# Da1yuqin/TCDiff

Hardware: AMD Instinct MI355X
Metric: sampled clips/sec (3 dancers x 150 frames, 1000 DDPM steps) (higher is better)
Workload: dtype bf16; 1 GPU; batch=16 clips/GPU, 3 dancers x 150 frames, 1000 DDPM steps (p_sample_loop, CFG w=2, cosine schedule), bf16, 1xMI355X; clips_per_gpu=16, ddpm_steps=1000

## Files before the change

### tcdiff_amd/csrc/chain.hip

```cpp
#include "common.h"
#include "tcdiff_hip.h"

#include "chain_core.h"

#ifdef CH_ABLATE_ROWLAT
#define CH_RP_NEXT(rp, nt) do { } while (0)
#else
#define CH_RP_NEXT(rp, nt) rp_issue(rp, nt)
#endif

template <int HH, int MT, int NT, bool SELF = false>
DEVINL void cross_attention(const f32x4_t (&qacc)[NT][MT], const tcdiff_chain_args& a, int m0, int Mv, int lblk, char* abuf,
                            int wave, int lane) {
#ifdef CH_XATT_ONEPASS
    constexpr bool PARK = !SELF;
#else
    constexpr bool PARK = false;
#endif
    constexpr bool ONEPASS = SELF || PARK;
    constexpr int NPS = ONEPASS ? 1 : (MT == 4 ? 2 : 1), NML = ONEPASS ? MT : (MT == 1 ? 1 : 2);
    lane = fresh_v(lane);
    wave = fresh_s(wave) * (NT / 4) + HH;
    const int c = lane & 15, g = lane >> 4;
    const int M = Mv, L = a.L, nkt = SELF ? a.sa_nkt : a.nkt, Lk = SELF ? a.L : a.Lk;
    const float qs = a.scale_q * CH_LOG2E;
    u32x4 qf[MT][2];
    if constexpr (SELF) {
        const u32x4* qsrc = reinterpret_cast<const u32x4*>(a.sa_q) + ((long)(lblk * 8 + wave) * 8) * 64 + lane;
#pragma unroll
        for (int mt = 0; mt < MT; ++mt)
#pragma unroll
            for (int s = 0; s < 2; ++s) qf[mt][s] = qsrc[(mt * 2 + s) * 64];
    } else {
#pragma unroll
        for (int mt = 0; mt < MT; ++mt)
#pragma unroll
            for (int s = 0; s < 2; ++s) {
                const f32x4_t lo = qacc[4 * HH + 2 * s][mt], hi = qacc[4 * HH + 2 * s + 1][mt];
                qf[mt][s][0] = pack_bf2(lo[0] * qs, lo[1] * qs);
                qf[mt][s][1] = pack_bf2(lo[2] * qs, lo[3] * qs);
                qf[mt][s][2] = pack_bf2(hi[0] * qs, hi[1] * qs);
                qf[mt][s][3] = pack_bf2(hi[2] * qs, hi[3] * qs);
            }
    }
    char* qpark = abuf + (CH_H1C - CH_ABUF) + wave * 8192 + lane * 16;
    if constexpr (PARK) {
#pragma unroll
        for (int mt = 0; mt < MT; ++mt)
#pragma unroll
            for (int s = 0; s < 2; ++s) *reinterpret_cast<u32x4*>(qpark + (mt * 2 + s) * 1024) = qf[mt][s];
    }
    u32x4 ones = {0x3F803F80u, 0x3F803F80u, 0x3F803F80u, 0x3F803F80u};
    asm volatile("" : "+v"(ones));
    const unsigned voff = (unsigned)lane * 16u;
    const __amdgpu_buffer_rsrc_t kr = __builtin_amdgcn_make_buffer_rsrc(const_cast<void*>(SELF ? a.sa_kf : a.kf), 0, -1, 0x00020000);
    const __amdgpu_buffer_rsrc_t vr = __builtin_amdgcn_make_buffer_rsrc(const_cast<void*>(SELF ? a.sa_vf : a.vf), 0, -1, 0x00020000);
    auto ld_tile = [&](const __amdgpu_buffer_rsrc_t& r, unsigned so, u32x4 (&f)[4]) {
#pragma unroll
        for (int i = 0; i < 4; ++i) f[i] = __builtin_bit_cast(u32x4, __builtin_amdgcn_raw_buffer_load_b128(r, voff + 1024u * i, so, 0));
    };
#pragma unroll
    for (int ps = 0; ps < NPS; ++ps) {
        int ra = m0 + 16 * NML * ps, rb = ra + 16 * NML - 1;
        ra = ra < M ? ra : M - 1;
        rb = rb < M ? rb : M - 1;
        const int sa = ra / L, sb = rb / L;
        int my_seq[NML];
#pragma unroll
        for (int ml = 0; ml < NML; ++ml) {
            int mrow = m0 + 16 * NML * ps + 16 * ml + c;
            mrow = mrow < M ? mrow : M - 1;
            my_seq[ml] = mrow / L;
        }
#pragma unroll 1
        for (int seq = sa; seq <= sb; ++seq) {
            const int kv = SELF ? seq : seq < a.n_shared ? 0 : seq - a.n_shared + (a.n_shared > 0 ? 1 : 0);
            const unsigned so0 = (unsigned)((kv * a.H + wave) * nkt) * 4096u;
            f32x4_t o[4][NML];
#pragma unroll
            for (int dt = 0; dt < 4; ++dt)
#pragma unroll
                for (int ml = 0; ml < NML; ++ml) o[dt][ml] = f32x4_t{0, 0, 0, 0};
            f32x4_t lacc[NML];
            float m_run[NML], nb[NML];
#pragma unroll
            for (int ml = 0; ml < NML; ++ml) {
                m_run[ml] = -INFINITY;
                nb[ml] = 0.0f;
                lacc[ml] = f32x4_t{0, 0, 0, 0};
            }
            u32x4 kn[4];
            ld_tile(kr, so0, kn);
#pragma unroll 1
            for (int kt = 0; kt < nkt; ++kt) {
                u32x4 kc[4], vc[4];
#pragma unroll
                for (int i = 0; i < 4; ++i) kc[i] = kn[i];
                ld_tile(vr, so0 + (unsigned)kt * 4096u, vc);
                const int nx = kt + 1 < nkt ? kt + 1 : kt;
                if constexpr (!PARK) ld_tile(kr, so0 + (unsigned)nx * 4096u, kn);
                f32x4_t s0[NML], s1[NML];
#pragma unroll
                for (int ml = 0; ml < NML; ++ml) {
                    const int mt = NML * ps + ml;
                    s0[ml] = s1[ml] = f32x4_t{nb[ml], nb[ml], nb[ml], nb[ml]};
                    u32x4 q0 = qf[mt][0], q1 = qf[mt][1];
                    if constexpr (PARK) {
                        char* qp = qpark;
                        asm volatile("" : "+v"(qp));
                        q0 = *reinterpret_cast<const u32x4*>(qp + (mt * 2) * 1024);
                        q1 = *reinterpret_cast<const u32x4*>(qp + (mt * 2 + 1) * 1024);
                    }
                    mma16(s0[ml], kc[0], q0);
                    mma16(s1[ml], kc[2], q0);
                    mma16(s0[ml], kc[1], q1);
                    mma16(s1[ml], kc[3], q1);
                }
                if constexpr (PARK) {
#pragma unroll
                    for (int ml = 0; ml < NML; ++ml) asm volatile("" : "+v"(s0[ml]), "+v"(s1[ml]));
                    ld_tile(kr, so0 + (unsigned)nx * 4096u, kn);
                }
                if (kt * 32 + 32 > Lk) {
#pragma unroll
                    for (int ml = 0; ml < NML; ++ml)
#pragma unroll
                        for (int j = 0; j < 4; ++j) {
                            if (kt * 32 + 4 * g + j >= Lk) s0[ml][j] = -INFINITY;
                            if (kt * 32 + 16 + 4 * g + j >= Lk) s1[ml][j] = -INFINITY;
                        }
                }
                float lm[NML];
                bool hot = kt == 0;
#pragma unroll
                for (int ml = 0; ml < NML; ++ml) {
                    lm[ml] = lane_max8(s0[ml], s1[ml], -INFINITY);
                    hot = hot || lm[ml] > CH_ATT_THR;
                }
                if (__builtin_amdgcn_ballot_w64(hot) != 0) {
#pragma unroll
                    for (int ml = 0; ml < NML; ++ml) {
                        const float mx = ar4_max(lm[ml]);
                        const float m_new = (kt == 0 || mx > CH_ATT_THR) ? fmaxf(m_run[ml], mx - nb[ml]) : m_run[ml];
                        const float shift = m_new + nb[ml];
                        const float alpha = __builtin_amdgcn_exp2f(m_run[ml] - m_new);
                        m_run[ml] = m_new;
                        nb[ml] = -m_new;
#pragma unroll
                        for (int j = 0; j < 4; ++j) {
                            lacc[ml][j] *= alpha;
                            s0[ml][j] -= shift;
                            s1[ml][j] -= shift;
                        }
#pragma unroll
                        for (int dt = 0; dt < 4; ++dt)
#pragma unroll
                            for (int j = 0; j < 4; ++j) o[dt][ml][j] *= alpha;
                    }
                }
#pragma unroll
                for (int ml = 0; ml < NML; ++ml) {
#pragma unroll
                    for (int j = 0; j < 4; ++j) {
                        s0[ml][j] = __builtin_amdgcn_exp2f(s0[ml][j]);
                        s1[ml][j] = __builtin_amdgcn_exp2f(s1[ml][j]);
                    }
                    u32x4 pf;
                    pf[0] = pack_bf2(s0[ml][0], s0[ml][1]);
                    pf[1] = pack_bf2(s0[ml][2], s0[ml][3]);
                    pf[2] = pack_bf2(s1[ml][0], s1[ml][1]);
                    pf[3] = pack_bf2(s1[ml][2], s1[ml][3]);
#pragma unroll
                    for (int dt = 0; dt < 4; ++dt) mma16(o[dt][ml], vc[dt], pf);
                    mma16(lacc[ml], ones, pf);
                }
            }
#pragma unroll
            for (int ml = 0; ml < NML; ++ml) {
                const float lsum = lacc[ml][0];
                if (my_seq[ml] == seq) {
                    const float inv = __builtin_amdgcn_rcpf(lsum);
                    const int mt = NML * ps + ml;
#pragma unroll
                    for (int dt = 0; dt < 4; ++dt) {
                        uint2 pk;
                        pk.x = pack_bf2(o[dt][ml][0] * inv, o[dt][ml][1] * inv);
                        pk.y = pack_bf2(o[dt][ml][2] * inv, o[dt][ml][3] * inv);
                        *reinterpret_cast<uint2*>(abuf + wave * 8192 + act_wr_off(lane, dt) + mt * 2048) = pk;
                    }
                }
            }
        }
    }
}

#ifdef CH_STAMP
#ifndef CH_STAMP_BLOCK
#define CH_STAMP_BLOCK 0
#endif
#define CH_T(i) do { if (m0 == 64 * CH_STAMP_BLOCK && (threadIdx.x & 63) == 0 && (MODE == TC_CHAIN_B || MODE == TC_CHAIN_FULL)) \
        reinterpret_cast<unsigned long long*>(a.h_out)[(threadIdx.x >> 6) * 64 + (i)] = __builtin_amdgcn_s_memrealtime(); } while (0)
#define CH_TC(i) do { if (m0 == 64 * CH_STAMP_BLOCK && (threadIdx.x & 63) == 0 && (MODE == TC_CHAIN_B || MODE == TC_CHAIN_FULL)) \
        reinterpret_cast<unsigned long long*>(a.h_out)[(threadIdx.x >> 6) * 64 + (i)] = __builtin_amdgcn_s_memtime(); } while (0)
#else
#define CH_TC(i) do { } while (0)
#define CH_T(i) do { } while (0)
#endif

template <int MODE, int MT, int NT, int BRK>
DEVINL void chain_body(const tcdiff_chain_args& a) {
    constexpr int BR = BRK;
    constexpr int NW = ChW<NT>::NW, NTH = 64 * NW, RD = ChW<NT>::D;
    constexpr bool HAS_A = MODE == TC_CHAIN_A || MODE == TC_CHAIN_FULL || MODE == TC_CHAIN_FULL_LAST;
    constexpr bool FULL = MODE == TC_CHAIN_FULL || MODE == TC_CHAIN_FULL_LAST;
    constexpr bool LAST = MODE == TC_CHAIN_B_LAST || MODE == TC_CHAIN_FULL_LAST;
    constexpr bool FRONT = MODE == TC_CHAIN_FRONT;
    extern __shared__ __attribute__((aligned(16))) char smem[];
    const int tid = threadIdx.x, lane = tid & 63;
    const int wave = __builtin_amdgcn_readfirstlane(tid >> 6);
    const int c = lane & 15, g = lane >> 4;
    const int dn = FRONT ? a.dn : 1;
    const int dancer = FRONT ? (int)(blockIdx.x % (unsigned)dn) : 0;
    const int lblk = FRONT ? (int)(blockIdx.x / (unsigned)dn) : xcd_remap(blockIdx.x, gridDim.x);
    const bool seqcut = !FRONT && a.seq_blocks;
    const int nbs = seqcut ? (a.L + BR - 1) / BR : 1;
    const int bseq = seqcut ? lblk / nbs : 0, bis = seqcut ? lblk - bseq * nbs : 0;
    const int m0 = seqcut ? bseq * a.L + bis * BR : lblk * BR;
    CH_T(0);
    CH_TC(60);
    const int Mtot = a.M, L = a.L;
    const int M = seqcut ? (bseq + 1) * L : Mtot;
    char* abuf = smem + CH_ABUF;
    char* h1c = smem + CH_H1C;
    float* scr = reinterpret_cast<float*>(smem + CH_SCR);
    char* cfilm = smem + CH_FILM;
    char* cvec = smem + CH_VEC;

    const int seq0 = (m0 < M ? m0 : M - 1) / L;
    const int seq_last = (Mtot - 1) / L;
    const int seqb = (seq0 + 1) * L;
    struct Rows { int mc[MT], sidx[MT]; };
    auto rows = [&]() {
        Rows r;
        const int cc = fresh_v(c);
#pragma unroll
        for (int mt = 0; mt < MT; ++mt) {
            const int m = m0 + 16 * mt + cc;
            r.mc[mt] = m < M ? m : M - 1;
            r.sidx[mt] = r.mc[mt] >= seqb ? 1 : 0;
        }
        return r;
    };
    auto positions = [&](const Rows& r, int (&pos)[MT]) {
#pragma unroll
        for (int mt = 0; mt < MT; ++mt)
            pos[mt] = FRONT ? (r.mc[mt] * dn + dancer) % L : r.mc[mt] - (r.sidx[mt] ? seqb : seqb - L);
    };
    constexpr int CF = 512 / NTH, CV = (768 + NTH - 1) / NTH;
    struct Consts { f32x4_t f[CF], v[CV]; };
    auto fetch_consts = [&](const float* film, const float* const (&vec)[6]) {
        Consts k;
#pragma unroll
        for (int j = 0; j < CF; ++j) {
            const int idx = j * NTH + tid;
            int sq = seq0 + (idx >> 8);
            sq = sq < seq_last ? sq : seq_last;
            k.f[j] = film ? ld4(film + (long)sq * a.film_ld + (idx & 255) * 4) : f32x4_t{0, 0, 0, 0};
        }
#pragma unroll
        for (int j = 0; j < CV; ++j) {
            const int idx = j * NTH + tid;
            const int vi = idx >> 7;
            const float* p0 = vi == 0 ? vec[0] : vi == 1 ? vec[1] : vi == 2 ? vec[2] : vi == 3 ? vec[3] : vi == 4 ? vec[4] : vi == 5 ? vec[5] : nullptr;
            k.v[j] = p0 ? ld4(p0 + (idx & 127) * 4) : f32x4_t{0, 0, 0, 0};
        }
        return k;
    };
    auto store_consts = [&](const Consts& k) {
#pragma unroll
        for (int j = 0; j < CF; ++j) *reinterpret_cast<f32x4_t*>(cfilm + (j * NTH + tid) * 16) = k.f[j];
#pragma unroll
        for (int j = 0; j < CV; ++j)
            if (j * NTH + tid < 768) *reinterpret_cast<f32x4_t*>(cvec + (j * NTH + tid) * 16) = k.v[j];
    };
    auto vecp = [&](int slot) { return cvec + slot * 2048; };
    const float* fcb_film = FULL ? a.filmb : a.film;
    const float* n3_g = FULL ? a.n3_g : a.n2_g;
    const float* n3_b = FULL ? a.n3_b : a.n2_b;

    constexpr int NWL = 2 * MT < NW ? 2 * MT : NW;
    const bool self_att = FULL && NT == 4 && a.sa_q != nullptr;
    WStreamT<NT> ws;
    ws.rsrc = __builtin_amdgcn_make_buffer_rsrc(
        const_cast<char*>(reinterpret_cast<const char*>(a.wstream)) + ((long)dancer * NW + wave) * a.n_stages * ChW<NT>::STAGE, 0,
        a.n_stages * ChW<NT>::STAGE, 0x00020000);
    ws.voff = (unsigned)lane * 16u;
    ws.pos = 0;
    ws.last = (unsigned)a.n_stages - 1;
    auto ring_fill = [&]() {
#pragma unroll
        for (int i = 0; i < RD; ++i) ws_load(ws, i, (unsigned)i);
    };
    f32x4_t acc[NT][MT];
    if constexpr (FULL && NT == 4) {
        if (self_att) {
            cross_attention<0, MT, NT, true>(acc, a, m0, M, lblk, abuf, wave, lane);
            ring_fill();
        }
    }
    if (!self_att) {
        if (wave < NWL) {
#pragma unroll
            for (int kt = 0; kt < (FRONT ? 16 : 8); ++kt)
                stage_glds<16 * MT, NWL>(abuf + kt * 8192, reinterpret_cast<const char*>(a.A) + kt * TC_ROWB, FRONT ? 2048 : 1024, m0,
                                    M, a.a_mod, wave, lane);
        }
        ring_fill();
    }
    if (FRONT) {
        const float* const v[6] = {a.b3 + 512 * dancer, a.nn_g, a.nn_b, nullptr, nullptr, nullptr};
        store_consts(fetch_consts(nullptr, v));
    } else {
        const float* const v[6] = {nullptr, nullptr, a.n2_g, a.n2_b, nullptr, nullptr};
        store_consts(fetch_consts(a.film, v));
    }
    __builtin_amdgcn_s_waitcnt(0x0F70);
    __syncthreads();
    CH_T(1);


    float nmr[MT], rstd[MT];
    RowPipe<MT> rp;
    const long xrows = (long)Mtot * dn;
    const __amdgpu_buffer_rsrc_t xo = f32_buffer(a.xout, xrows * 512);
    Consts nxt;

    auto fc_epilogue = [&](float eps, int stamp) {
        CH_T(stamp);
        row_stats(acc, scr, wave, lane, eps, nmr, rstd);
        CH_T(stamp + 1);
        const int gg = fresh_v(g), wv = fresh_s(wave);
        const Rows rw = rows();
        const int cb0 = col_base_bytes<NT>(wv, gg);
        auto body = [&](int nt, int mt, const f32x4_t& G, const f32x4_t& Bv) {
            const f32x4_t x4 = rp.q[nt & 1][mt];
            f32x4_t o;
#pragma unroll
            for (int t = 0; t < 4; ++t) {
                float v = fmaf(fmaf(acc[nt][mt][t], rstd[mt], nmr[mt]), G[t], Bv[t]);
                v = x4[t] + v;
                acc[nt][mt][t] = v;
                o[t] = v;
            }
#ifdef CH_STORE_EARLY
            cb_store<NT>(xo, Mtot, wv, nt, rw.mc[mt], gg, o);
#endif
        };
        int fb[MT];
#pragma unroll
        for (int mt = 0; mt < MT; ++mt) {
            fb[mt] = rw.sidx[mt] * 4096 + cb0;
            asm volatile("" : "+v"(fb[mt]));
        }
#pragma unroll
        for (int nt = 0; nt < NT; ++nt) {
#pragma unroll
            for (int mt = 0; mt < MT; ++mt)
                body(nt, mt, lds4b(cfilm + fb[mt], 64 * nt), lds4b(cfilm + fb[mt], 2048 + 64 * nt));
            if (nt + 2 < NT) CH_RP_NEXT(rp, nt + 2);
            CH_FENCE();
        }
#ifndef CH_STORE_EARLY
#pragma unroll
        for (int nt = 0; nt < NT; ++nt)
#pragma unroll
            for (int mt = 0; mt < MT; ++mt) cb_store<NT>(xo, Mtot, wv, nt, rw.mc[mt], gg, acc[nt][mt]);
#endif
    };
    auto xres_start = [&]() {
        const Rows rw = rows();
        int rr[MT];
#pragma unroll
        for (int mt = 0; mt < MT; ++mt) rr[mt] = a.xres_mod > 0 ? rw.mc[mt] % a.xres_mod : rw.mc[mt];
        rp_start<NT>(rp, a.xres, rr, a.xres_rowmajor ? 0 : (a.xres_mod > 0 ? a.xres_mod : Mtot), a.xres_mod > 0 ? a.xres_mod : Mtot, wave,
                     fresh_v(g));
    };
    auto xout_start = [&]() {
        const Rows rw = rows();
        rp_start<NT>(rp, a.xout, rw.mc, Mtot, Mtot, wave, fresh_v(g));
    };
    auto rope_start = [&]() {
        const Rows rw = rows();
        int pos[MT];
        positions(rw, pos);
        rp_start<NT>(rp, a.rope, pos, a.rope_rows, a.rope_rows, wave, fresh_v(g));
    };

    if (HAS_A) {
        zero(acc);
        phase_n512<16, false, MT, NT>(acc, abuf, ws, lane);
        CH_T(2);
        xres_start();
        fc_epilogue(a.ln_eps, 40);
        CH_T(3);
        if (FULL) {
            const float* const v[6] = {nullptr, nullptr, n3_g, n3_b, nullptr, nullptr};
            nxt = fetch_consts(fcb_film, v);
        }
        rope_start();
        row_stats(acc, scr + 1024, wave, lane, a.n2_eps, nmr, rstd);
        CH_T(4);
        norm_to_lds<true, MT, NT>(acc, nmr, rstd, vecp(2), vecp(3), rp, abuf, wave, lane, nullptr);
        lds_barrier();
        CH_T(34);
        if (FULL) store_consts(nxt);
        zero(acc);
        if (!FULL) {
            phase_n512<16, false, MT, NT>(acc, abuf, ws, lane);
            store_heads<true, MT, NT>(acc, a.q_out, a.scale_q, L, a.Lp, a.H, m0, M, wave, lane, smem);
            return;
        }
#ifdef CH_STAMP
        {
            unsigned long long* sp = nullptr;
            if (m0 == 64 * CH_STAMP_BLOCK) {
                sp = reinterpret_cast<unsigned long long*>(a.h_out) + 512 + wave * 32;
                if (lane == 0) sp[16] = __builtin_amdgcn_s_memtime();
            }
            phase_n512<16, false, MT, NT>(acc, abuf, ws, lane, sp);
        }
#else
        phase_n512<16, false, MT, NT>(acc, abuf, ws, lane);
#endif
        CH_T(35);
        lds_barrier();
#ifndef CH_ABLATE_XATTN
        cross_attention<0>(acc, a, m0, M, lblk, abuf, wave, lane);
        if constexpr (NT == 8) cross_attention<1>(acc, a, m0, M, lblk, abuf, wave, lane);
#endif
        CH_T(36);
        lds_barrier();
    }
    if constexpr (!FRONT) {
    zero(acc);
    phase_n512<16, false, MT, NT>(acc, abuf, ws, lane);
    if (FULL)
        xout_start();
    else
        xres_start();
    CH_T(37);
    fc_epilogue(a.ln_eps, 42);
    CH_T(38);
    row_stats(acc, scr + 1024, wave, lane, a.n2_eps, nmr, rstd);
    CH_T(39);
    {
        const float* const v[6] = {a.b1, a.b1 + 512, nullptr, a.n4_g, a.n4_b, nullptr};
        nxt = fetch_consts(a.film3, v);
    }
    norm_to_lds<false, MT, NT>(acc, nmr, rstd, vecp(2), vecp(3), rp, abuf, wave, lane, nullptr);
    lds_barrier();
    store_consts(nxt);
    lds_barrier();
    CH_T(5);
    zero(acc);
#pragma unroll 1
    for (int ch = 0; ch < 4; ++ch) {
        f32x4_t a1[NT / 2][MT];
#pragma unroll
        for (int nt = 0; nt < NT / 2; ++nt)
#pragma unroll
            for (int mt = 0; mt < MT; ++mt) a1[nt][mt] = f32x4_t{0, 0, 0, 0};
        phase_ff1<MT, NT>(a1, abuf, ws, lane);
        CH_T(6 + 4 * ch);
        char* hb = h1c + (ch & 1) * 32768;
        CH_T(7 + 4 * ch);
        {
            const int nb = 256 * ch + 8 * NT * wave + 4 * g;
#pragma unroll
            for (int nt = 0; nt < NT / 2; ++nt) {
                const f32x4_t b4 = lds4(cvec, nb + 16 * nt);
                const int wo = ((8 * NT * wave + 16 * nt) >> 6) * 8192 + act_wr_off(lane, 0, ((8 * NT * wave + 16 * nt) & 63) >> 3);
#pragma unroll
                for (int mt = 0; mt < MT; ++mt) {
                    float v[4];
#pragma unroll
                    for (int t = 0; t < 4; ++t) v[t] = a1[nt][mt][t] + b4[t];
#ifndef CH_ABLATE_GELU
                    act4_ct<ACT_GELU>(v, ACT_GELU);
#endif
                    uint2 pk;
                    pk.x = pack_bf2(v[0], v[1]);
                    pk.y = pack_bf2(v[2], v[3]);
                    *reinterpret_cast<uint2*>(hb + wo + mt * 2048) = pk;
                }
            }
        }
        lds_barrier();
        CH_T(8 + 4 * ch);
        phase_n512<8, false, MT, NT>(acc, hb, ws, lane);
        CH_T(9 + 4 * ch);
    }
    xout_start();
    {
        const int cb2 = col_base_bytes<NT>(fresh_s(wave), fresh_v(g));
        const Rows rw = rows();
        auto body2 = [&](int nt, int mt, const f32x4_t& G, const f32x4_t& Bv) {
            const f32x4_t x4 = rp.q[nt & 1][mt];
#pragma unroll
            for (int t = 0; t < 4; ++t) acc[nt][mt][t] = x4[t] + fmaf(acc[nt][mt][t], G[t], Bv[t]);
            asm volatile("" ::"v"(acc[nt][mt][0]), "v"(acc[nt][mt][1]), "v"(acc[nt][mt][2]), "v"(acc[nt][mt][3]));
        };
        int fb2[MT];
#pragma unroll
        for (int mt = 0; mt < MT; ++mt) {
            fb2[mt] = rw.sidx[mt] * 4096 + cb2;
            asm volatile("" : "+v"(fb2[mt]));
        }
#pragma unroll
        for (int nt = 0; nt < NT; ++nt) {
#pragma unroll
            for (int mt = 0; mt < MT; ++mt)
                body2(nt, mt, lds4b(cfilm + fb2[mt], 64 * nt), lds4b(cfilm + fb2[mt], 2048 + 64 * nt));
            if (nt + 2 < NT) CH_RP_NEXT(rp, nt + 2);
            CH_FENCE();
        }
    }
    CH_T(22);
    {
        const float* const v[6] = {a.b3, a.nn_g, a.nn_b, nullptr, nullptr, nullptr};
        nxt = fetch_consts(nullptr, v);
    }
    row_stats(acc, scr, wave, lane, a.n4_eps, nmr, rstd);
    CH_T(23);
    norm_to_lds<false, MT, NT>(acc, nmr, rstd, vecp(3), vecp(4), rp, abuf, wave, lane, nullptr);
    lds_barrier();
    store_consts(nxt);
    }
    CH_T(24);
    zero(acc);
    if (FRONT)
        phase_n512<32, false, MT, NT>(acc, abuf, ws, lane);
    else if (LAST)
        phase_n512<16, true, MT, NT>(acc, abuf, ws, lane);
    else
        phase_n512<16, false, MT, NT>(acc, abuf, ws, lane);
    CH_T(25);
    lds_barrier();
#ifndef CH_STORE_EARLY
    if (!LAST) rope_start();
#endif
    {
        const int g3 = fresh_v(g);
        const int cb3 = col_base_bytes<NT>(fresh_s(wave), g3);
        const Rows rw = rows();
#pragma unroll
        for (int nt = 0; nt < NT; ++nt) {
            const int n = 16 * NT * wave + 16 * nt + 4 * g3;
            const f32x4_t b4 = lds4b(vecp(0) + cb3, 64 * nt);
#pragma unroll
            for (int mt = 0; mt < MT; ++mt) {
                f32x4_t o;
#pragma unroll
                for (int t = 0; t < 4; ++t) {
                    acc[nt][mt][t] += b4[t];
                    o[t] = acc[nt][mt][t];
                }
                if (LAST && a.out_ld > 0) {
                    if (n < a.out_ld)
                        *reinterpret_cast<f32x4_t*>(reinterpret_cast<float*>(a.h_out) + (long)rw.mc[mt] * a.out_ld + n) = o;
                } else if (LAST) {
                    uint2 pk;
                    pk.x = pack_bf2(o[0], o[1]);
                    pk.y = pack_bf2(o[2], o[3]);
                    *reinterpret_cast<uint2*>(reinterpret_cast<uint16_t*>(a.h_out) + (long)rw.mc[mt] * 512 + n) = pk;
                } else {
                    cb_store<NT>(xo, xrows, wave, nt, rw.mc[mt] * dn + dancer, g3, o);
                }
            }
            CH_FENCE();
        }
    }
    if (LAST) return;
    CH_T(26);
#ifdef CH_STORE_EARLY
    rope_start();
#endif
    row_stats(acc, scr, wave, lane, a.nn_eps, nmr, rstd);
    CH_T(27);
    norm_to_lds<true, MT, NT>(acc, nmr, rstd, vecp(1), vecp(2), rp, abuf, wave, lane, smem + CH_ABUF2);
    lds_barrier();
    CH_T(28);
    zero(acc);
    phase_n512<16, false, MT, NT>(acc, abuf, ws, lane);
    CH_T(29);
    constexpr bool FRAG = !FRONT && NT == 4;
    bool frag_out = false;
    if constexpr (FRAG) frag_out = a.qf_out != nullptr;
    if constexpr (FRAG) {
        if (frag_out) store_qfrag<MT>(acc, a.qf_out, a.scale_q, lblk, wave, lane);
    }
    if (!frag_out) store_heads<true, MT, NT>(acc, a.q_out, a.scale_q, L, a.Lp, a.H, m0, M, wave, lane, smem, dn, dancer);
    zero(acc);
    phase_n512<16, false, MT, NT>(acc, abuf, ws, lane);
    CH_T(30);
    if constexpr (FRAG) {
        if (frag_out) store_kfrag<MT>(acc, a.kf_out, bseq, bis * BR, a.out_nkt, wave, lane);
    }
    if (!frag_out) store_heads<false, MT, NT>(acc, a.k_out, 1.0f, L, a.Lp, a.H, m0, M, wave, lane, smem, dn, dancer);
    CH_T(31);
    zero(acc);
    if constexpr (FRAG) {
        if (frag_out) {
            phase_n512<16, true, MT, NT, true>(acc, smem + CH_ABUF2, ws, lane);
            CH_T(32);
            store_vfrag<MT>(acc, a.vf_out, bseq, bis * BR, a.out_nkt, L, wave, lane);
            CH_T(33);
            CH_TC(61);
            return;
        }
    }
    phase_n512<16, true, MT, NT>(acc, smem + CH_ABUF2, ws, lane);
    CH_T(32);
    store_heads<false, MT, NT>(acc, a.v_out, 1.0f, L, a.Lp, a.H, m0, M, wave, lane, smem, dn, dancer);
    CH_T(33);
    CH_TC(61);
}

template <int MODE, int MT, int NT>
__global__ __launch_bounds__(2048 / NT) void chain_kernel(tcdiff_chain_args a) {
    constexpr bool DUAL = (MODE == TC_CHAIN_FULL || MODE == TC_CHAIN_FULL_LAST) && NT == 4 && MT > 1;
    if constexpr (DUAL) {
        if (a.seq_blocks) {
            const int lblk = xcd_remap(blockIdx.x, gridDim.x);
            const int nbs = (a.L + 16 * MT - 1) / (16 * MT);
            if (a.L - (lblk % nbs) * 16 * MT <= 16) {
                chain_body<MODE, 1, NT, 16 * MT>(a);
                return;
            }
        }
    }
    chain_body<MODE, MT, NT, 16 * MT>(a);
}

static bool al16(const void* p) { return (reinterpret_cast<uintptr_t>(p) & 15) == 0; }

extern "C" int tcdiff_chain(const tcdiff_chain_args* a, hipStream_t stream) {
    if (!a || a->M <= 0 || a->L <= 0 || !a->A || !a->wstream) return TC_ERR_ARG;
    const bool front = a->mode == TC_CHAIN_FRONT;
    if (!front && a->L < 64) return TC_ERR_UNSUPPORTED;
    const int want = a->mode == TC_CHAIN_A ? 32 : a->mode == TC_CHAIN_B ? 144 : a->mode == TC_CHAIN_B_LAST ? 96 :
                     a->mode == TC_CHAIN_FULL ? 176 : a->mode == TC_CHAIN_FULL_LAST ? 128 : front ? 80 : -1;
    if (want < 0 || a->n_stages != want) return TC_ERR_ARG;
    if (a->out_ld < 0 || a->out_ld % 4 || a->out_ld > 512) return TC_ERR_ARG;
    const void* ptrs[] = {a->A, a->wstream, a->film, a->xres, a->xout, a->n2_g, a->n2_b, a->rope,
                          a->q_out, a->b1, a->film3, a->n4_g, a->n4_b, a->b3, a->nn_g, a->nn_b, a->k_out,
                          a->v_out, a->h_out, a->filmb, a->n3_g, a->n3_b, a->kf, a->vf};
    for (const void* p : ptrs)
        if (p && !al16(p)) return TC_ERR_ALIGN;
    if (front) {
        if (a->dn <= 0 || a->L % a->dn || a->L / a->dn < 8 || !a->b3 || !a->nn_g || !a->nn_b || !a->rope || !a->xout ||
            !a->q_out || !a->k_out || !a->v_out || a->H != 8 || a->Lp <= 0 || a->a_mod != 0)
            return TC_ERR_ARG;
        if ((long)a->M * 2048 >= (1L << 32)) return TC_ERR_ARG;
    } else {
        if (!a->film || a->film_ld % 4 || !a->xres || !a->xout || !a->n2_g || !a->n2_b) return TC_ERR_ARG;
        if ((long)(a->a_mod > 0 ? a->a_mod : a->M) * 1024 >= (1L << 32)) return TC_ERR_ARG;
    }
    const bool has_a = a->mode == TC_CHAIN_A || a->mode == TC_CHAIN_FULL || a->mode == TC_CHAIN_FULL_LAST;
    const bool has_b = a->mode != TC_CHAIN_A && !front;
    const bool full = a->mode == TC_CHAIN_FULL || a->mode == TC_CHAIN_FULL_LAST;
    const bool last = a->mode == TC_CHAIN_B_LAST || a->mode == TC_CHAIN_FULL_LAST;
    if (has_a && (!a->rope || a->H != 8)) return TC_ERR_ARG;
    if (a->mode == TC_CHAIN_A && (!a->q_out || a->Lp <= 0)) return TC_ERR_ARG;
    if (has_b && (!a->b1 || !a->film3 || !a->n4_g || !a->n4_b || !a->b3)) return TC_ERR_ARG;
    const bool frag_out = a->qf_out || a->kf_out || a->vf_out;
    if (has_b && !last &&
        (!a->rope || !a->nn_g || !a->nn_b || (!frag_out && (!a->q_out || !a->k_out || !a->v_out)) || a->H != 8 || a->Lp <= 0))
        return TC_ERR_ARG;
    if (last && !a->h_out) return TC_ERR_ARG;
    if (full && (!a->filmb || !a->n3_g || !a->n3_b || !a->kf || !a->vf || a->nkt <= 0 ||
                 a->Lk <= 0 || a->Lk > 32 * a->nkt || a->n_shared < 0))
        return TC_ERR_ARG;
    if (a->seq_blocks && (front || a->M % a->L)) return TC_ERR_ARG;
    if (a->sa_q && (!full || !a->seq_blocks || !a->sa_kf || !a->sa_vf || a->sa_nkt <= 0 || a->L > 32 * a->sa_nkt)) return TC_ERR_ARG;
    if (frag_out && (!a->qf_out || !a->kf_out || !a->vf_out || !has_b || last || !a->seq_blocks || a->out_nkt <= 0 ||
                     a->L > 32 * a->out_nkt))
        return TC_ERR_ARG;
    if ((a->sa_q || frag_out) && a->nw == 4) return TC_ERR_UNSUPPORTED;
    for (const void* p : {a->sa_q, a->sa_kf, a->sa_vf, (const void*)a->qf_out, (const void*)a->kf_out, (const void*)a->vf_out})
        if (p && !al16(p)) return TC_ERR_ALIGN;
    if (a->sa_q && (long)(a->M / a->L) * 8 * a->sa_nkt * 4096 >= (1L << 32)) return TC_ERR_ARG;
    static tc_dev_state dev_state;
    const int n_cu = tc_device_once(dev_state, [](int) {
#define CH_FN(M_, NT_) reinterpret_cast<const void*>(chain_kernel<M_, 4, NT_>), reinterpret_cast<const void*>(chain_kernel<M_, 2, NT_>), \
                        reinterpret_cast<const void*>(chain_kernel<M_, 1, NT_>)
        const void* fns[27] = {CH_FN(TC_CHAIN_A, 4), CH_FN(TC_CHAIN_B, 4), CH_FN(TC_CHAIN_B_LAST, 4), CH_FN(TC_CHAIN_FULL, 4),
                               CH_FN(TC_CHAIN_FULL_LAST, 4), CH_FN(TC_CHAIN_FRONT, 4),
                               CH_FN(TC_CHAIN_FULL, 8), CH_FN(TC_CHAIN_FULL_LAST, 8), CH_FN(TC_CHAIN_FRONT, 8)};
#undef CH_FN
        for (const void* f : fns) {
            hipError_t e = hipFuncSetAttribute(f, hipFuncAttributeMaxDynamicSharedMemorySize, CH_SMEM);
            if (e != hipSuccess) return e;
        }
        return hipSuccess;
    });
    if (n_cu < 0) return n_cu;
    const int units = front ? a->dn : 1;
    int mt = a->mt;
    if (mt == 0) mt = ((a->M + 15) / 16) * units <= n_cu ? 1 : ((a->M + 31) / 32) * units <= n_cu ? 2 : 4;
    if (mt != 1 && mt != 2 && mt != 4) return TC_ERR_ARG;
    dim3 grid(((a->M + 16 * mt - 1) / (16 * mt)) * units);
    if (a->seq_blocks) grid.x = (a->M / a->L) * ((a->L + 16 * mt - 1) / (16 * mt));
    if (a->nw != 0 && a->nw != 4 && a->nw != 8) return TC_ERR_ARG;
    const bool four = a->nw == 4;
    if (four && !(full || front)) return TC_ERR_UNSUPPORTED;
#define CH_LAUNCH_NT(MODE_, NT_)                                                                                              \
    do {                                                                                                                      \
        if (mt == 4) hipLaunchKernelGGL((chain_kernel<MODE_, 4, NT_>), grid, dim3(2048 / NT_), CH_SMEM, stream, *a);          \
        else if (mt == 2) hipLaunchKernelGGL((chain_kernel<MODE_, 2, NT_>), grid, dim3(2048 / NT_), CH_SMEM, stream, *a);     \
        else hipLaunchKernelGGL((chain_kernel<MODE_, 1, NT_>), grid, dim3(2048 / NT_), CH_SMEM, stream, *a);                  \
    } while (0)
#define CH_LAUNCH(MODE_) CH_LAUNCH_NT(MODE_, 4)
#define CH_LAUNCH2(MODE_) do { if (four) CH_LAUNCH_NT(MODE_, 8); else CH_LAUNCH_NT(MODE_, 4); } while (0)
    switch (a->mode) {
        case TC_CHAIN_FRONT: CH_LAUNCH2(TC_CHAIN_FRONT); break;
        case TC_CHAIN_A: CH_LAUNCH(TC_CHAIN_A); break;
        case TC_CHAIN_B: CH_LAUNCH(TC_CHAIN_B); break;
        case TC_CHAIN_B_LAST: CH_LAUNCH(TC_CHAIN_B_LAST); break;
        case TC_CHAIN_FULL: CH_LAUNCH2(TC_CHAIN_FULL); break;
        default: CH_LAUNCH2(TC_CHAIN_FULL_LAST); break;
    }
#undef CH_LAUNCH
#undef CH_LAUNCH2
#undef CH_LAUNCH_NT
    TC_CHECK_LAUNCH();
    return TC_OK;
}
```

Before: 14.37 clips/s.

## Spread front-chain A staging across all waves and defer residual store

In the FRONT mode, the A-tile staging into LDS is now split across all wave groups instead of only the first NWL waves. The constant fetch is issued before the weight ring fill, and the wait only drains down to the ring loads rather than all outstanding loads. Block-to-dancer mapping now goes through the XCD remap. The residual output store is moved after the layernorm-to-LDS step so it overlaps with later work. Timing stamps are extended to the FRONT mode. The goal is a shorter prologue and hidden store latency, at the cost of more complex wait-count logic that depends on the ring depth.

```diff
diff --git a/tcdiff_amd/csrc/chain.hip b/tcdiff_amd/csrc/chain.hip
--- a/tcdiff_amd/csrc/chain.hip
+++ b/tcdiff_amd/csrc/chain.hip
@@ -198,9 +198,11 @@
 #ifndef CH_STAMP_BLOCK
 #define CH_STAMP_BLOCK 0
 #endif
-#define CH_T(i) do { if (m0 == 64 * CH_STAMP_BLOCK && (threadIdx.x & 63) == 0 && (MODE == TC_CHAIN_B || MODE == TC_CHAIN_FULL)) \
+#define CH_STAMP_ON (m0 == 64 * CH_STAMP_BLOCK && (threadIdx.x & 63) == 0 && \
+                     (MODE == TC_CHAIN_B || MODE == TC_CHAIN_FULL || (MODE == TC_CHAIN_FRONT && dancer == 0)))
+#define CH_T(i) do { if (CH_STAMP_ON) \
         reinterpret_cast<unsigned long long*>(a.h_out)[(threadIdx.x >> 6) * 64 + (i)] = __builtin_amdgcn_s_memrealtime(); } while (0)
-#define CH_TC(i) do { if (m0 == 64 * CH_STAMP_BLOCK && (threadIdx.x & 63) == 0 && (MODE == TC_CHAIN_B || MODE == TC_CHAIN_FULL)) \
+#define CH_TC(i) do { if (CH_STAMP_ON) \
         reinterpret_cast<unsigned long long*>(a.h_out)[(threadIdx.x >> 6) * 64 + (i)] = __builtin_amdgcn_s_memtime(); } while (0)
 #else
 #define CH_TC(i) do { } while (0)
@@ -220,8 +222,9 @@
     const int wave = __builtin_amdgcn_readfirstlane(tid >> 6);
     const int c = lane & 15, g = lane >> 4;
     const int dn = FRONT ? a.dn : 1;
-    const int dancer = FRONT ? (int)(blockIdx.x % (unsigned)dn) : 0;
-    const int lblk = FRONT ? (int)(blockIdx.x / (unsigned)dn) : xcd_remap(blockIdx.x, gridDim.x);
+    const int lid = xcd_remap(blockIdx.x, gridDim.x);
+    const int dancer = FRONT ? (int)((unsigned)lid % (unsigned)dn) : 0;
+    const int lblk = FRONT ? (int)((unsigned)lid / (unsigned)dn) : lid;
     const bool seqcut = !FRONT && a.seq_blocks;
     const int nbs = seqcut ? (a.L + BR - 1) / BR : 1;
     const int bseq = seqcut ? lblk / nbs : 0, bis = seqcut ? lblk - bseq * nbs : 0;
@@ -308,24 +311,37 @@
             ring_fill();
         }
     }
-    if (!self_att) {
-        if (wave < NWL) {
-#pragma unroll
-            for (int kt = 0; kt < (FRONT ? 16 : 8); ++kt)
-                stage_glds<16 * MT, NWL>(abuf + kt * 8192, reinterpret_cast<const char*>(a.A) + kt * TC_ROWB, FRONT ? 2048 : 1024, m0,
-                                    M, a.a_mod, wave, lane);
-        }
+    if constexpr (FRONT) {
+        constexpr int NG = NW / NWL;
+        const int grp = wave / NWL, wl = wave % NWL;
+#pragma unroll
+        for (int kt = 0; kt < 16 / NG; ++kt)
+            stage_glds<16 * MT, NWL>(abuf + (kt * NG + grp) * 8192, reinterpret_cast<const char*>(a.A) + (kt * NG + grp) * TC_ROWB, 2048,
+                                     m0, M, a.a_mod, wl, lane);
+        const float* const v[6] = {a.b3 + 512 * dancer, a.nn_g, a.nn_b, nullptr, nullptr, nullptr};
+        const Consts k0 = fetch_consts(nullptr, v);
         ring_fill();
-    }
-    if (FRONT) {
-        const float* const v[6] = {a.b3 + 512 * dancer, a.nn_g, a.nn_b, nullptr, nullptr, nullptr};
-        store_consts(fetch_consts(nullptr, v));
+        CH_T(44);
+        store_consts(k0);
+        constexpr int RING_LOADS = RD * NT;
+        static_assert(RING_LOADS == 16 || RING_LOADS == 32, "vmcnt immediate below");
+        __builtin_amdgcn_s_waitcnt(RING_LOADS == 16 ? 0x4F70 : 0x8F70);
+        __syncthreads();
     } else {
+        if (!self_att) {
+            if (wave < NWL) {
+#pragma unroll
+                for (int kt = 0; kt < 8; ++kt)
+                    stage_glds<16 * MT, NWL>(abuf + kt * 8192, reinterpret_cast<const char*>(a.A) + kt * TC_ROWB, 1024, m0, M, a.a_mod,
+                                             wave, lane);
+            }
+            ring_fill();
+        }
         const float* const v[6] = {nullptr, nullptr, a.n2_g, a.n2_b, nullptr, nullptr};
         store_consts(fetch_consts(a.film, v));
-    }
-    __builtin_amdgcn_s_waitcnt(0x0F70);
-    __syncthreads();
+        __builtin_amdgcn_s_waitcnt(0x0F70);
+        __syncthreads();
+    }
     CH_T(1);
 
 
@@ -549,6 +565,12 @@
 #ifndef CH_STORE_EARLY
     if (!LAST) rope_start();
 #endif
+#ifdef CH_STORE_EARLY
+    constexpr bool FRONT_LATE = false;
+#else
+    constexpr bool FRONT_LATE = FRONT;
+#endif
+    CH_T(45);
     {
         const int g3 = fresh_v(g);
         const int cb3 = col_base_bytes<NT>(fresh_s(wave), g3);
@@ -573,7 +595,7 @@
                     pk.x = pack_bf2(o[0], o[1]);
                     pk.y = pack_bf2(o[2], o[3]);
                     *reinterpret_cast<uint2*>(reinterpret_cast<uint16_t*>(a.h_out) + (long)rw.mc[mt] * 512 + n) = pk;
-                } else {
+                } else if (!FRONT_LATE) {
                     cb_store<NT>(xo, xrows, wave, nt, rw.mc[mt] * dn + dancer, g3, o);
                 }
             }
@@ -588,6 +610,14 @@
     row_stats(acc, scr, wave, lane, a.nn_eps, nmr, rstd);
     CH_T(27);
     norm_to_lds<true, MT, NT>(acc, nmr, rstd, vecp(1), vecp(2), rp, abuf, wave, lane, smem + CH_ABUF2);
+    if constexpr (FRONT_LATE) {
+        const int g3 = fresh_v(g), wv = fresh_s(wave);
+        const Rows rw = rows();
+#pragma unroll
+        for (int nt = 0; nt < NT; ++nt)
+#pragma unroll
+            for (int mt = 0; mt < MT; ++mt) cb_store<NT>(xo, xrows, wv, nt, rw.mc[mt] * dn + dancer, g3, acc[nt][mt]);
+    }
     lds_barrier();
     CH_T(28);
     zero(acc);
```

Measured after the change: 14.44 clips/s (median of 4 runs). About the same (+0.5%).
